# david-gimeno/tailored-avsr

Hardware: AMD Instinct MI355X
Metric: utterances/sec fwd+bwd, 12L tailored AV-Branchformer (Conv3d+ResNet-18 lip frontend, fusion, CTC+6L decoder), 4 s clips, batch 32/GPU (higher is better)
Workload: dtype f32

## Files before the change

profiles/gemm_trace.py:

```python
import ctypes as C
import os
import sys

ROOT = os.path.dirname(os.path.dirname(os.path.abspath(__file__)))
sys.path[:0] = [ROOT, os.path.join(ROOT, "tailored-avsr_amd")]
import numpy as np
import torch

from tavsr import _lib, ops

SHAPES = [("NT", 3168, 2048, 256, (4, 1)), ("NT", 3168, 2048, 256, (8, 1)), ("NT", 3168, 256, 2048, (4, 1)),
          ("NT", 3168, 256, 2048, (8, 4)), ("NT", 3168, 256, 2048, (8, 5)), ("NT", 3168, 256, 256, (4, 1)),
          ("NN", 3168, 256, 2048, (4, 1)), ("TN", 2048, 256, 3168, (4, 4))]


def pct(x):
    return " ".join(f"{np.percentile(x, q):7.2f}" for q in (0, 10, 50, 90, 100))


def main():
    L = _lib.lib()
    L.tavsr_gemm_trace_read.restype = C.c_int
    buf = np.zeros((1 << 15, 6), dtype=np.uint64)
    for mode, M, N, K, force in SHAPES:
        a = torch.randn(M, K, device="cuda")
        b = torch.randn(K, N, device="cuda")
        A = a.t().contiguous() if mode == "TN" else a
        B = b if mode != "NT" else b.t().contiguous()
        Cout = torch.empty(M, N, device="cuda")
        kw = dict(a_kmajor=mode == "TN", b_kmajor=mode != "NT")
        for _ in range(3):
            ops.gemm(M, N, K, A, A.stride(0), B, B.stride(0), Cout, N, force=force, **kw)
        torch.cuda.synchronize()
        L.tavsr_gemm_trace_read(buf.ctypes.data_as(C.c_void_p), buf.shape[0])
        ops.gemm(M, N, K, A, A.stride(0), B, B.stride(0), Cout, N, force=force, **kw)
        n = L.tavsr_gemm_trace_read(buf.ctypes.data_as(C.c_void_p), buf.shape[0])
        t = buf[:n, :4].astype(np.int64)
        t0 = t[:, 0].min()
        us = (t - t0) / 100.0
        hw = buf[:n, 4]
        xcc = (hw >> np.uint64(32)) & np.uint64(0xF)
        hwid = hw & np.uint64(0xFFFFFFFF)
        cu = (hwid >> np.uint64(8)) & np.uint64(0xF)
        sh = (hwid >> np.uint64(12)) & np.uint64(0x1)
        se = (hwid >> np.uint64(13)) & np.uint64(0x7)
        cuid = (xcc * np.uint64(8) + se) * np.uint64(32) + sh * np.uint64(16) + cu
        ncu = len(np.unique(cuid))
        per_cu = np.bincount(np.unique(cuid, return_inverse=True)[1])
        print(f"== {mode} M={M} N={N} K={K} cfg/split={force}: {n} workgroups on {ncu} CUs "
              f"(per CU min/med/max {per_cu.min()}/{int(np.median(per_cu))}/{per_cu.max()}), span {us[:, 3].max():.2f} us")
        print(f"   percentiles            {'p0':>7} {'p10':>7} {'p50':>7} {'p90':>7} {'p100':>7}")
        print(f"   start offset           {pct(us[:, 0])}")
        print(f"   prologue (first tile)  {pct(us[:, 1] - us[:, 0])}")
        print(f"   K loop                 {pct(us[:, 2] - us[:, 1])}")
        print(f"   epilogue               {pct(us[:, 3] - us[:, 2])}")
        print(f"   lifetime               {pct(us[:, 3] - us[:, 0])}")
        print(f"   end                    {pct(us[:, 3])}")
        cyc = buf[:n, 5].astype(np.float64)
        loop_us = np.maximum(us[:, 2] - us[:, 1], 1e-3)
        nk = max(1, (K // force[1]) // 32 - 1)
        print(f"   K-loop cycles/K-step   {pct(cyc / nk)}   shader clock GHz {pct(cyc / loop_us / 1e3)}", flush=True)


if __name__ == "__main__":
    main()
```

tailored-avsr_amd/csrc/gemm.hip:

```cpp
#include <algorithm>
#include <type_traits>

#include <cstdlib>
#include "common.h"

namespace tavsr {

typedef float f32x16 __attribute__((ext_vector_type(16)));

struct GemmArgs {
  tavsr_gemm_desc d;
  int kchunk;
  int nsplit;
  int tiles_m, tiles_n;
  int vec_epi;
  int zmap;
};

template <int V>
__global__ __launch_bounds__(256) void splitk_epilogue_kernel(const GemmArgs args) {
  const tavsr_gemm_desc& d = args.d;
  const int64_t mn = (int64_t)d.M * d.N;
  const int nbatch = d.nb1 * d.nb2;
  const int64_t i = ((int64_t)blockIdx.x * 256 + threadIdx.x) * V;
  const int z = blockIdx.y, z1 = z / d.nb2, z2 = z % d.nb2;
  if (d.a_rowsum && z == 0 && i < d.M) {
    const float* rs = d.ws + (int64_t)args.nsplit * nbatch * mn;
    for (int q = 0; q < V && i + q < d.M; ++q) {
      float v = 0.f;
      for (int s = 0; s < args.nsplit; ++s) v += rs[(int64_t)s * d.M + i + q];
      d.a_rowsum[i + q] = d.alpha * v;
    }
  }
  if (i >= mn) return;
  const int m = (int)(i / d.N), n = (int)(i % d.N);
  float v[V];
#pragma unroll
  for (int q = 0; q < V; ++q) v[q] = 0.f;
  const float* p = d.ws + (int64_t)z * mn + i;
#pragma unroll 4
  for (int s = 0; s < args.nsplit; ++s) {
    if (V == 4) {
      const float4 t = *reinterpret_cast<const float4*>(p + (int64_t)s * nbatch * mn);
      v[0] += t.x; v[1 % V] += t.y; v[2 % V] += t.z; v[3 % V] += t.w;
    } else {
      v[0] += p[(int64_t)s * nbatch * mn];
    }
  }
  const int64_t o = z1 * d.sC1 + z2 * d.sC2 + (int64_t)m * d.ldc + n;
  const int64_t ro = z1 * d.sR1 + z2 * d.sR2 + (int64_t)m * d.ldr + n;
  uint32_t keep[4] = {1u, 1u, 1u, 1u};
  float inv_keep = 1.f;
  if (V == 4 && d.drop_p > 0.f) {
    const uint64_t sd = d.drop_seed[0], ctr = (d.drop_offset >> 2) + (uint64_t)(i >> 2);
// ... 68 lines not shown
        if (gk < K) {
          const float* p = g + (int64_t)gk * ld + gr;
          if (VEC && gr + 3 < nrows) {
            val = *reinterpret_cast<const float4*>(p);
          } else {
            if (gr + 0 < nrows) val.x = p[0];
            if (gr + 1 < nrows) val.y = p[1];
            if (gr + 2 < nrows) val.z = p[2];
            if (gr + 3 < nrows) val.w = p[3];
          }
        }
      } else {
        if (gr < nrows) {
          const float* p = g + (int64_t)gr * ld + gk;
          if (VEC && gk + 3 < K) {
            val = *reinterpret_cast<const float4*>(p);
          } else {
            if (gk + 0 < K) val.x = p[0];
            if (gk + 1 < K) val.y = p[1];
            if (gk + 2 < K) val.z = p[2];
            if (gk + 3 < K) val.w = p[3];
          }
        }
      }
      r[i] = val;
    }
  }
  __device__ static __forceinline__ void store(float* __restrict__ s, int tid, const float4 (&r)[NV]) {
#pragma unroll
    for (int i = 0; i < NV; ++i) {
      int row, k;
      coords(tid + i * NT, row, k);
      *reinterpret_cast<float4*>(s + (KMAJOR ? k * T::LD + row : row * T::LD + k)) = r[i];
    }
  }
};

template <int ROWS, int BK, bool KMAJOR>
__device__ __forceinline__ void read_frag(const float* __restrict__ s, int row, int g, int lk, float (&f)[4]) {
  using T = Tile<ROWS, BK, KMAJOR>;
  if (KMAJOR) {
    const float* p = s + (g * 8 + 4 * lk) * T::LD + row;
#pragma unroll
    for (int j = 0; j < 4; ++j) f[j] = p[j * T::LD];
  } else {
    const float4 v = *reinterpret_cast<const float4*>(s + row * T::LD + g * 8 + 4 * lk);
    f[0] = v.x; f[1] = v.y; f[2] = v.z; f[3] = v.w;
  }
}

struct PosMajor {
  int n, H, W;
  int uni, base, rp;
  __device__ __forceinline__ void pos(int v, int& y, int& x) const {
    const int Hi = max(H - 2, 0), Wi = max(W - 2, 0), Hb = H - Hi, Wb = W - Wi;
    int u = v;
    if (u < Hi * Wi) { y = u / Wi + 1; x = u % Wi + 1; return; }
    u -= Hi * Wi;
    if (u < Hi * Wb) { y = u / Wb + 1; x = (u % Wb) ? W - 1 : 0; return; }
    u -= Hi * Wb;
    if (u < Hb * Wi) { y = (u / Wi) ? H - 1 : 0; x = u % Wi + 1; return; }
    u -= Hb * Wi;
    y = (u / Wb) ? H - 1 : 0;
    x = (u % Wb) ? W - 1 : 0;
  }
  __device__ __forceinline__ uint32_t taps(int y, int x) const {
    uint32_t mk = 0;
#pragma unroll
    for (int tap = 0; tap < 9; ++tap)
      mk |= (uint32_t)((unsigned)(y + tap / 3 - 1) < (unsigned)H && (unsigned)(x + tap % 3 - 1) < (unsigned)W) << tap;
    return mk;
  }
  __device__ __forceinline__ int row(int r) const {
    if (uni) return (r - base) * (H * W) + rp;
    const int v = r / n;
    int y, x;
    pos(v, y, x);
    return (r - v * n) * (H * W) + y * W + x;
  }
};

template <int TM, int TN, bool PM = false>
__device__ __forceinline__ void finish_tile(const tavsr_gemm_desc& d, int nsplit, f32x16 (&acc)[TM][TN],
                                            float (&asum)[TM], bool want_rowsum, int m0, int n0, int wm, int wn, int lr,
                                            int lk, int z1, int z2, int64_t coff, int zidx, const float* bias_pre = nullptr,
                                            const PosMajor* pm = nullptr) {
  if (want_rowsum) {
#pragma unroll
    for (int i = 0; i < TM; ++i) asum[i] += __shfl_xor(asum[i], 32, 64);
  }

  if (nsplit > 1) {
    const int64_t mn = (int64_t)d.M * d.N;
    const int nbatch = gridDim.y;
    float* slab = d.ws + ((int64_t)zidx * nbatch + blockIdx.y) * mn;
    float* rsum0 = d.ws + (int64_t)nsplit * nbatch * mn;
#pragma unroll
    for (int j = 0; j < TN; ++j) {
      const int n = n0 + wn * TN * 32 + j * 32 + lr;
      if (n >= d.N) continue;
#pragma unroll
      for (int i = 0; i < TM; ++i) {
        const int mb = m0 + wm * TM * 32 + i * 32 + 4 * lk;
#pragma unroll
        for (int r = 0; r < 16; ++r) {
          const int m = mb + (r & 3) + 8 * (r >> 2);
          if (m < d.M) slab[(int64_t)(PM ? pm->row(m) : m) * d.N + n] = acc[i][j][r];
        }
      }
    }
    if (want_rowsum && lk == 0) {
#pragma unroll
      for (int i = 0; i < TM; ++i) {
        const int m = m0 + wm * TM * 32 + i * 32 + lr;
        if (m < d.M) rsum0[(int64_t)zidx * d.M + m] = asum[i];
      }
    }
    return;
  }

  if (want_rowsum && lk == 0) {
#pragma unroll
    for (int i = 0; i < TM; ++i) {
      const int m = m0 + wm * TM * 32 + i * 32 + lr;
      if (m < d.M) d.a_rowsum[m] = d.alpha * asum[i];
    }
  }
  float* C = d.C + coff;
  float* Z = d.Z ? d.Z + coff : nullptr;
  const float* R = d.R ? d.R + z1 * d.sR1 + z2 * d.sR2 : nullptr;
  const float* DZ = d.DZ ? d.DZ + coff : nullptr;
#pragma unroll
  for (int j = 0; j < TN; ++j) {
// ... 808 lines not shown
      float* r0 = red + ((kw - 1) * WM * WN + w2) * PER * 64 + lane;
#pragma unroll
      for (int i = 0; i < TM; ++i)
#pragma unroll
        for (int j = 0; j < TN; ++j)
#pragma unroll
          for (int r = 0; r < 16; ++r) r0[((i * TN + j) * 16 + r) * 64] = acc[i][j][r];
#pragma unroll
      for (int i = 0; i < TM; ++i) rsum[(((kw - 1) * WM * WN + w2) * TM + i) * 64 + lane] = asum[i];
    }
    __syncthreads();
    if (kw > 0) return;
#pragma unroll
    for (int s2 = 0; s2 < KW - 1; ++s2) {
      const float* r0 = red + (s2 * WM * WN + w2) * PER * 64 + lane;
#pragma unroll
      for (int i = 0; i < TM; ++i)
#pragma unroll
        for (int j = 0; j < TN; ++j)
#pragma unroll
          for (int r = 0; r < 16; ++r) acc[i][j][r] += r0[((i * TN + j) * 16 + r) * 64];
#pragma unroll
      for (int i = 0; i < TM; ++i) asum[i] += rsum[((s2 * WM * WN + w2) * TM + i) * 64 + lane];
    }
  }
  if (KW == 1 && vec_epi) {
    static_assert(KW > 1 || BM * BN <= S * STAGE, "the output tile image must fit in the staging ring");
    if (want_rowsum) {
#pragma unroll
      for (int i = 0; i < TM; ++i) asum[i] += __shfl_xor(asum[i], 32, 64);
      if (lk == 0) {
#pragma unroll
        for (int i = 0; i < TM; ++i) {
          const int m = m0 + wm * TM * 32 + i * 32 + lr;
          if (m < d.M) {
            if (nsplit > 1) (d.ws + (int64_t)nsplit * gridDim.y * d.M * d.N)[(int64_t)zidx * d.M + m] = asum[i];
            else d.a_rowsum[m] = d.alpha * asum[i];
          }
        }
      }
    }
    finish_tile_vec<BM, BN, NT, TM, TN, PM && CONV == 1>(d, nsplit, acc, smem, m0, n0, wm, wn, lr, lk, z1, z2, coff, tid, zidx, &pm);
  } else {
    finish_tile<TM, TN, PM && CONV == 1>(d, nsplit, acc, asum, want_rowsum, m0, n0, wm, wn, lr, lk, z1, z2, coff, zidx, bpre, &pm);
  }
#ifdef TAVSR_GEMM_TRACE
  __builtin_amdgcn_s_waitcnt(0);
  TAVSR_TRACE_AT(3)
  if (tid == 0) {
    unsigned int slot = atomicAdd(&g_trace_n, 1u);
    if (slot < (unsigned)kTraceMax) {
      for (int i = 0; i < 4; ++i) g_trace[slot][i] = tr_t[i];
      g_trace[slot][4] = ((unsigned long long)__builtin_amdgcn_s_getreg((31 << 11) | 20) << 32) | __builtin_amdgcn_s_getreg((31 << 11) | 4);
      g_trace[slot][5] = tr_c[2] - tr_c[1];
    }
  }
#endif
}

__device__ __forceinline__ int xcd_remap(int bid, int nwg) {
  const int xcd = bid & 7, q = nwg >> 3, r = nwg & 7;
  return (xcd < r ? xcd * (q + 1) : r * (q + 1) + (xcd - r) * q) + (bid >> 3);
}

template <int BM, int BN, int WM, int WN, int S, int MINW, bool AK, bool BKM, int KW = 1, int CONV = 0, bool PM = false>
__global__ __launch_bounds__(WM* WN * KW * 64, MINW)
void gemm_glds_kernel(const GemmArgs args) {
  int bid = xcd_remap(blockIdx.x, gridDim.x), zidx = blockIdx.z;
  if (args.zmap) {
    const int tiles = gridDim.x, l = blockIdx.x + tiles * blockIdx.z, j = l >> 3;
    zidx = (l & 7) + 8 * (j / tiles);
    bid = j % tiles;
  }
  glds_tile<BM, BN, WM, WN, S, AK, BKM, KW, CONV, PM>(args.d, args.kchunk, args.nsplit, args.tiles_n, bid, args.vec_epi != 0, zidx);
}

constexpr int kMaxGroup = 12;
struct GroupArgs {
  tavsr_gemm_desc d[kMaxGroup];
  int tile_start[kMaxGroup + 1];
  int tiles_n[kMaxGroup];
  int n;
  int vec_epi;
};

template <int BM, int BN, int WM, int WN, int S, int MINW, bool AK, bool BKM>
__global__ __launch_bounds__(WM* WN * 64, MINW)
void gemm_glds_grouped_kernel(const GroupArgs g) {
  const int bid = xcd_remap(blockIdx.x, gridDim.x);
  int pi = 0;
#pragma unroll
  for (int i = 1; i < kMaxGroup; ++i)
    if (i < g.n && bid >= g.tile_start[i]) pi = i;
  glds_tile<BM, BN, WM, WN, S, AK, BKM>(g.d[pi], g.d[pi].K, 1, g.tiles_n[pi], bid - g.tile_start[pi], g.vec_epi != 0, 0);
}

struct Cfg {
  int bm, bn, wm, wn, stages;
};
static const Cfg kCfgs[] = {
    {128, 128, 2, 2, 3},
    {128, 128, 2, 4, 3},
    {128, 64, 2, 2, 3},
    {64, 128, 2, 2, 3},
    {64, 64, 2, 2, 3},
    {64, 64, 2, 2, 4},
    {128, 64, 2, 2, 4},
    {64, 64, 2, 2, 3},
    {64, 64, 2, 2, 2},
};
constexpr int kNumCfgs = sizeof(kCfgs) / sizeof(kCfgs[0]);
constexpr int kFallbackCfg = 9;

template <typename F>
static int launch_layout(const tavsr_gemm_desc& d, F&& f) {
  if (!d.a_kmajor && !d.b_kmajor) return f(std::false_type{}, std::false_type{});
  if (!d.a_kmajor && d.b_kmajor) return f(std::false_type{}, std::true_type{});
  if (d.a_kmajor && d.b_kmajor) return f(std::true_type{}, std::true_type{});
  return f(std::true_type{}, std::false_type{});
}

struct LnTail {
  const float* gamma; const float* beta; float eps; float* out; int64_t ld;
};
static const LnTail* g_ln_tail = nullptr;
// ... 51 lines not shown
      const float a = x[q].x - mean, b = x[q].y - mean, c = x[q].z - mean, e = x[q].w - mean;
      sq += (a * a + b * b) + (c * c + e * e);
    }
  }
  const float rstd = rsqrtf(wave_sum(sq) / (float)d.N + ln.eps);
#pragma unroll
  for (int q = 0; q < Q; ++q) {
    const int c4 = lane + 64 * q;
    if (c4 < n4) {
      const float4 g = *reinterpret_cast<const float4*>(ln.gamma + 4 * c4), b = *reinterpret_cast<const float4*>(ln.beta + 4 * c4);
      *reinterpret_cast<float4*>(ln.out + (int64_t)m * ln.ld + 4 * c4) =
          make_float4((x[q].x - mean) * rstd * g.x + b.x, (x[q].y - mean) * rstd * g.y + b.y, (x[q].z - mean) * rstd * g.z + b.z,
                      (x[q].w - mean) * rstd * g.w + b.w);
    }
  }
}

static int launch_epilogue(const GemmArgs& a, hipStream_t s) {
  const tavsr_gemm_desc& d = a.d;
  if (g_ln_tail) {
    hipLaunchKernelGGL(epilogue_ln_kernel, dim3(cdiv(d.M, 4)), dim3(256), 0, s, a, *g_ln_tail);
    TAVSR_LAUNCH_CHECK();
    return TAVSR_OK;
  }
  if (a.nsplit > 1) {
    const int64_t mn = (int64_t)d.M * d.N;
    if (d.N % 4 == 0)
      hipLaunchKernelGGL(splitk_epilogue_kernel<4>, dim3(cdiv(mn / 4, 256), d.nb1 * d.nb2), dim3(256), 0, s, a);
    else
      hipLaunchKernelGGL(splitk_epilogue_kernel<1>, dim3(cdiv(mn, 256), d.nb1 * d.nb2), dim3(256), 0, s, a);
    TAVSR_LAUNCH_CHECK();
  }
  return TAVSR_OK;
}

template <int BM, int BN, int WM, int WN, int S, int MINW, int KW = 1>
static int launch_glds(const tavsr_gemm_desc& d, int nsplit, int kchunk, hipStream_t s) {
  GemmArgs a{d, kchunk, nsplit, cdiv(d.M, BM), cdiv(d.N, BN), (int)vec_epi_ok(d)};
  dim3 grid(a.tiles_m * a.tiles_n, d.nb1 * d.nb2, nsplit);
  int rc = launch_layout(d, [&](auto ak, auto bk) {
    hipLaunchKernelGGL((gemm_glds_kernel<BM, BN, WM, WN, S, MINW, decltype(ak)::value, decltype(bk)::value, KW>), grid,
                       dim3(WM * WN * KW * 64), 0, s, a);
    TAVSR_LAUNCH_CHECK();
    return (int)TAVSR_OK;
  });
  return rc ? rc : launch_epilogue(a, s);
}

static bool conv_pm(const tavsr_gemm_desc& d) {
  return d.conv_posmajor && (d.conv_mode == 1 || d.conv_mode == 2) && d.conv_stride <= 1 && (d.conv_taps == 0 || d.conv_taps == 9) &&
         (d.conv_mode == 2 || !d.a_rowsum);
}

static int launch_conv(const tavsr_gemm_desc& d, int nsplit, int kchunk, hipStream_t s) {
  const int ve = (int)vec_epi_ok(d);
  constexpr int wide = 1;
  constexpr int dw_wide = 1;
  constexpr int zmap_on = 1;
  const int zmap = zmap_on && (d.conv_mode == 2 || d.conv_mode == 5 || d.conv_mode == 7) && nsplit >= 8 && nsplit % 8 == 0;
  if (d.conv_mode == 6 || d.conv_mode == 7) {
    GemmArgs a6{d, kchunk, nsplit, cdiv(d.M, 64), cdiv(d.N, 64), ve, zmap};
    const dim3 grid6(a6.tiles_m * a6.tiles_n, 1, nsplit);
    constexpr int st3 = 2;
    constexpr int tile128 = 0;
    if (d.conv_mode == 6 && tile128) {
      GemmArgs a7{d, kchunk, nsplit, cdiv(d.M, 128), cdiv(d.N, 64), ve, 0};
      hipLaunchKernelGGL((gemm_glds_kernel<128, 64, 2, 2, 2, 3, false, false, 1, 6>), dim3(a7.tiles_m * a7.tiles_n, 1, 1), dim3(256), 0, s, a7);
      TAVSR_LAUNCH_CHECK();
      return TAVSR_OK;
    }
    if (d.conv_mode == 6 && st3 == 3)
      hipLaunchKernelGGL((gemm_glds_kernel<64, 64, 2, 2, 3, 3, false, false, 1, 6>), grid6, dim3(256), 0, s, a6);
    else if (d.conv_mode == 6)
      hipLaunchKernelGGL((gemm_glds_kernel<64, 64, 2, 2, 2, 5, false, false, 1, 6>), grid6, dim3(256), 0, s, a6);
    else if (st3 == 3)
      hipLaunchKernelGGL((gemm_glds_kernel<64, 64, 2, 2, 3, 3, true, true, 1, 7>), grid6, dim3(256), 0, s, a6);
    else
      hipLaunchKernelGGL((gemm_glds_kernel<64, 64, 2, 2, 2, 5, true, true, 1, 7>), grid6, dim3(256), 0, s, a6);
    TAVSR_LAUNCH_CHECK();
    return launch_epilogue(a6, s);
  }
  if (d.conv_mode == 4 || d.conv_mode == 5) {
    GemmArgs a4{d, kchunk, nsplit, cdiv(d.M, 64), cdiv(d.N, 64), ve, zmap};
    const dim3 grid4(a4.tiles_m * a4.tiles_n, 1, nsplit);
    if (d.conv_mode == 4)
      hipLaunchKernelGGL((gemm_glds_kernel<64, 64, 2, 2, 2, 5, false, false, 1, 4>), grid4, dim3(256), 0, s, a4);
    else
      hipLaunchKernelGGL((gemm_glds_kernel<64, 64, 2, 2, 2, 5, true, true, 1, 5>), grid4, dim3(256), 0, s, a4);
    TAVSR_LAUNCH_CHECK();
    return launch_epilogue(a4, s);
  }
  const bool pm = conv_pm(d) && d.conv_mode == 1, pm2 = conv_pm(d) && d.conv_mode == 2;
  if (d.conv_mode == 1 && !d.b_kmajor && nsplit == 1 && wide && d.N % 128 == 0) {
    GemmArgs a2{d, kchunk, nsplit, cdiv(d.M, 64), cdiv(d.N, 128), (int)vec_epi_ok(d)};
    if (pm)
      hipLaunchKernelGGL((gemm_glds_kernel<64, 128, 2, 2, 2, 3, false, false, 1, 1, true>), dim3(a2.tiles_m * a2.tiles_n, 1, 1), dim3(256), 0, s, a2);
    else
      hipLaunchKernelGGL((gemm_glds_kernel<64, 128, 2, 2, 2, 3, false, false, 1, 1>), dim3(a2.tiles_m * a2.tiles_n, 1, 1), dim3(256), 0, s, a2);
    TAVSR_LAUNCH_CHECK();
    return TAVSR_OK;
  }
  if (d.conv_mode == 2 && dw_wide && d.M % 128 == 0) {
    GemmArgs a2{d, kchunk, nsplit, cdiv(d.M, 128), cdiv(d.N, 64), (int)vec_epi_ok(d), zmap};
    if (pm2)
      hipLaunchKernelGGL((gemm_glds_kernel<128, 64, 2, 2, 2, 3, true, true, 1, 2, true>), dim3(a2.tiles_m * a2.tiles_n, 1, nsplit), dim3(256), 0, s, a2);
    else
      hipLaunchKernelGGL((gemm_glds_kernel<128, 64, 2, 2, 2, 3, true, true, 1, 2>), dim3(a2.tiles_m * a2.tiles_n, 1, nsplit), dim3(256), 0, s, a2);
    TAVSR_LAUNCH_CHECK();
    return launch_epilogue(a2, s);
  }
  GemmArgs a{d, kchunk, nsplit, cdiv(d.M, 64), cdiv(d.N, 64), ve, zmap};
  dim3 grid(a.tiles_m * a.tiles_n, 1, nsplit);
  if (pm && !d.b_kmajor)
    hipLaunchKernelGGL((gemm_glds_kernel<64, 64, 2, 2, 2, 5, false, false, 1, 1, true>), grid, dim3(256), 0, s, a);
  else if (pm)
    hipLaunchKernelGGL((gemm_glds_kernel<64, 64, 2, 2, 2, 5, false, true, 1, 1, true>), grid, dim3(256), 0, s, a);
  else if (d.conv_mode == 1 && !d.b_kmajor)
    hipLaunchKernelGGL((gemm_glds_kernel<64, 64, 2, 2, 2, 5, false, false, 1, 1>), grid, dim3(256), 0, s, a);
  else if (d.conv_mode == 1)
    hipLaunchKernelGGL((gemm_glds_kernel<64, 64, 2, 2, 2, 5, false, true, 1, 1>), grid, dim3(256), 0, s, a);
  else if (pm2)
    hipLaunchKernelGGL((gemm_glds_kernel<64, 64, 2, 2, 2, 5, true, true, 1, 2, true>), grid, dim3(256), 0, s, a);
  else
    hipLaunchKernelGGL((gemm_glds_kernel<64, 64, 2, 2, 2, 5, true, true, 1, 2>), grid, dim3(256), 0, s, a);
  TAVSR_LAUNCH_CHECK();
  return launch_epilogue(a, s);
}

static int launch_fallback(const tavsr_gemm_desc& d, bool vec, int nsplit, int kchunk, hipStream_t s) {
  GemmArgs a{d, kchunk, nsplit, cdiv(d.M, 64), cdiv(d.N, 64), 0};
  dim3 grid(a.tiles_m * a.tiles_n, d.nb1 * d.nb2, nsplit);
  int rc = launch_layout(d, [&](auto ak, auto bk) {
    if (vec)
      hipLaunchKernelGGL((gemm_kernel<64, 64, 32, 2, 2, 2, 4, decltype(ak)::value, decltype(bk)::value, true>), grid,
                         dim3(256), 0, s, a);
    else
      hipLaunchKernelGGL((gemm_kernel<64, 64, 32, 2, 2, 2, 4, decltype(ak)::value, decltype(bk)::value, false>), grid,
                         dim3(256), 0, s, a);
    TAVSR_LAUNCH_CHECK();
    return (int)TAVSR_OK;
  });
  return rc ? rc : launch_epilogue(a, s);
}

static int launch_tail(const tavsr_gemm_desc& d, int nsplit, int kchunk, hipStream_t s) {
  GemmArgs a{d, kchunk, nsplit, cdiv(d.M, 64), cdiv(d.N, 64), (int)vec_epi_ok(d)};
  dim3 grid(a.tiles_m * a.tiles_n, d.nb1 * d.nb2, nsplit);
  int rc = launch_layout(d, [&](auto ak, auto bk) {
    hipLaunchKernelGGL((gemm_glds_kernel<64, 64, 2, 2, 2, 5, decltype(ak)::value, decltype(bk)::value, 1, 3>), grid, dim3(256), 0, s, a);
    TAVSR_LAUNCH_CHECK();
    return (int)TAVSR_OK;
  });
  return rc ? rc : launch_epilogue(a, s);
}

static int launch(int cfg, const tavsr_gemm_desc& d, bool vec, int nsplit, int kchunk, hipStream_t s) {
  switch (cfg) {
    case 0: return launch_glds<128, 128, 2, 2, 3, 1>(d, nsplit, kchunk, s);
    case 1: return launch_glds<128, 128, 2, 4, 3, 2>(d, nsplit, kchunk, s);
    case 2: return launch_glds<128, 64, 2, 2, 3, 2>(d, nsplit, kchunk, s);
    case 3: return launch_glds<64, 128, 2, 2, 3, 2>(d, nsplit, kchunk, s);
    case 4: return launch_glds<64, 64, 2, 2, 3, 3>(d, nsplit, kchunk, s);
    case 5: return launch_glds<64, 64, 2, 2, 4, 2>(d, nsplit, kchunk, s);
    case 6: return launch_glds<128, 64, 2, 2, 4, 1>(d, nsplit, kchunk, s);
    case 7: return launch_glds<64, 64, 2, 2, 3, 4, 2>(d, nsplit, kchunk, s);
    case 8: return launch_glds<64, 64, 2, 2, 2, 5>(d, nsplit, kchunk, s);
    default: return launch_fallback(d, vec, nsplit, kchunk, s);
  }
}

// ... 263 lines not shown
extern "C" int tavsr_gemm_grouped(const tavsr_gemm_desc* descs, int32_t n, tavsr_stream_t stream) {
  using namespace tavsr;
  TAVSR_REQUIRE(descs != nullptr && n >= 1 && n <= kMaxGroup, TAVSR_EINVAL, "tavsr_gemm_grouped: 1..%d problems", kMaxGroup);
  GroupArgs g;
  g.n = n;
  int total = 0;
  for (int i = 0; i < n; ++i) {
    tavsr_gemm_desc d = descs[i];
    if (d.nb1 <= 0) d.nb1 = 1;
    if (d.nb2 <= 0) d.nb2 = 1;
    TAVSR_REQUIRE(d.A && d.B && d.C && d.M > 0 && d.N > 0 && d.K > 0, TAVSR_EINVAL, "tavsr_gemm_grouped: bad problem %d", i);
    TAVSR_REQUIRE(d.a_kmajor == descs[0].a_kmajor && d.b_kmajor == descs[0].b_kmajor, TAVSR_EUNSUPPORTED,
                  "tavsr_gemm_grouped: all problems must share one layout");
    TAVSR_REQUIRE(d.nb1 * d.nb2 == 1 && d.drop_p == 0.f, TAVSR_EUNSUPPORTED, "tavsr_gemm_grouped: unbatched problems without epilogue dropout only");
    const bool vec = aligned16(d.A) && aligned16(d.B) && d.lda % 4 == 0 && d.ldb % 4 == 0;
    TAVSR_REQUIRE(glds_ok(d, vec), TAVSR_EUNSUPPORTED,
                  "tavsr_gemm_grouped: problem %d needs the predicated kernel (alignment / K %% 32 / rows %% 4)", i);
    if (d.R == nullptr) { d.ldr = 0; d.sR1 = d.sR2 = 0; }
    g.d[i] = d;
    g.tile_start[i] = total;
    g.tiles_n[i] = cdiv(d.N, 64);
    total += cdiv(d.M, 64) * g.tiles_n[i];
  }
  for (int i = n; i <= kMaxGroup; ++i) g.tile_start[i] = total;
  g.vec_epi = 1;
  for (int i = 0; i < n; ++i) g.vec_epi &= (int)vec_epi_ok(g.d[i]);
  hipStream_t s = static_cast<hipStream_t>(stream);
  int rc = launch_layout(descs[0], [&](auto ak, auto bk) {
    hipLaunchKernelGGL((gemm_glds_grouped_kernel<64, 64, 2, 2, 2, 5, decltype(ak)::value, decltype(bk)::value>), dim3(total),
                       dim3(256), 0, s, g);
    TAVSR_LAUNCH_CHECK();
    return (int)TAVSR_OK;
  });
  return rc;
}

extern "C" int tavsr_gemm_tune(const tavsr_gemm_desc* dp, int32_t cfg, int32_t nsplit, tavsr_stream_t stream) {
  return tavsr::run(dp, cfg, nsplit, static_cast<hipStream_t>(stream));
}

extern "C" int64_t tavsr_gemm_ws(const tavsr_gemm_desc* dp) {
  using namespace tavsr;
  if (!dp) return 0;
  tavsr_gemm_desc d = *dp;
  if (d.nb1 <= 0) d.nb1 = 1;
  if (d.nb2 <= 0) d.nb2 = 1;
  if (d.M <= 0 || d.N <= 0) return 0;
  const bool vec = aligned16(d.A) && aligned16(d.B) && d.lda % 4 == 0 && d.ldb % 4 == 0 && d.sA1 % 4 == 0 &&
                   d.sA2 % 4 == 0 && d.sB1 % 4 == 0 && d.sB2 % 4 == 0;
  Plan p = d.conv_mode != 0 ? plan_conv(d, true) : plan(d, true, glds_ok(d, vec) || tail_ok(d, vec));
  return ws_floats_for(d, p.nsplit);
}

#ifdef TAVSR_GEMM_TRACE
extern "C" int tavsr_gemm_trace_read(unsigned long long* out, int max_rows) {
  unsigned int n = 0;
  if (hipDeviceSynchronize() != hipSuccess) return -1;
  if (hipMemcpyFromSymbol(&n, HIP_SYMBOL(tavsr::g_trace_n), sizeof(n)) != hipSuccess) return -1;
  int rows = (int)(n < (unsigned)tavsr::kTraceMax ? n : tavsr::kTraceMax);
  if (rows > max_rows) rows = max_rows;
  if (rows > 0 && hipMemcpyFromSymbol(out, HIP_SYMBOL(tavsr::g_trace), (size_t)rows * 6 * sizeof(unsigned long long)) != hipSuccess) return -1;
  n = 0;
  if (hipMemcpyToSymbol(HIP_SYMBOL(tavsr::g_trace_n), &n, sizeof(n)) != hipSuccess) return -1;
  return rows;
}
#endif
```

tailored-avsr_amd/tavsr/ops.py:

```python
from __future__ import annotations

import ctypes as C
import os
from typing import Optional, Sequence

import torch

from . import _lib as L
from ._lib import ACT, AttnDesc, GemmDesc, check, lib, ptr, require_cuda, stream

f32 = torch.float32


def empty(*shape, like: Optional[torch.Tensor] = None, dtype=f32, device=None):
    dev = like.device if like is not None else (device if device is not None else "cuda")
    return torch.empty(shape, dtype=dtype, device=dev)


_addr = L.addr


class GemmProfile:

    def __init__(self, by_shape: bool = False):
# ... 1402 lines not shown
    dx = torch.empty_like(x)
    dg, db = empty(Cn, like=x), empty(Cn, like=x)
    ws = empty(lib().tavsr_bn_ws(M, Cn), like=x)
    check(lib().tavsr_bn_bwd_pooled(ptr(dpool), ptr(idx), ptr(x), ptr(mean), ptr(rstd), ptr(gamma), ptr(beta), ptr(dx), ptr(dg), ptr(db), N,
                                    H, W, Cn, ACT[act], ptr(ws), stream()), "tavsr_bn_bwd_pooled")
    return dx, dg, db


def maxpool3x3s2_fwd(x, N, H, W, Cn):
    Ho, Wo = conv_out(H, 3, 2, 1), conv_out(W, 3, 2, 1)
    y = empty(N * Ho * Wo, Cn, like=x)
    idx = torch.empty((N * Ho * Wo, Cn), dtype=torch.uint8, device=x.device)
    check(lib().tavsr_maxpool3x3s2_fwd(ptr(x), ptr(y), ptr(idx), N, H, W, Cn, stream()), "tavsr_maxpool3x3s2_fwd")
    return y, idx, Ho, Wo


def bn_act_maxpool3x3s2_fwd(z, mean, rstd, gamma, beta, act, N, H, W, Cn):
    Ho, Wo = conv_out(H, 3, 2, 1), conv_out(W, 3, 2, 1)
    require_cuda(z, mean, rstd, gamma, beta)
    y = empty(N * Ho * Wo, Cn, like=z)
    idx = torch.empty((N * Ho * Wo, Cn), dtype=torch.uint8, device=z.device)
    check(lib().tavsr_bn_act_maxpool3x3s2_fwd(ptr(z), ptr(mean), ptr(rstd), ptr(gamma), ptr(beta), ACT[act], ptr(y), ptr(idx), N, H, W, Cn,
                                              stream()), "tavsr_bn_act_maxpool3x3s2_fwd")
    return y, idx, Ho, Wo


def maxpool3x3s2_bwd(dy, idx, N, H, W, Cn):
    dx = empty(N * H * W, Cn, like=dy)
    check(lib().tavsr_maxpool3x3s2_bwd(ptr(dy), ptr(idx), ptr(dx), N, H, W, Cn, stream()), "tavsr_maxpool3x3s2_bwd")
    return dx


def avgpool_fwd(x, N, P, Cn):
    y = empty(N, Cn, like=x)
    check(lib().tavsr_avgpool_fwd(ptr(x), ptr(y), N, P, Cn, stream()), "tavsr_avgpool_fwd")
    return y


def avgpool_bwd(dy, N, P, Cn):
    dx = empty(N * P, Cn, like=dy)
    check(lib().tavsr_avgpool_bwd(ptr(dy), ptr(dx), N, P, Cn, stream()), "tavsr_avgpool_bwd")
    return dx


def conv_wflip(w2d, cout, cin):
    require_cuda(w2d)
    out = empty(cin, 9 * cout, like=w2d)
    check(lib().tavsr_conv_wflip(ptr(w2d), ptr(out), cout, cin, stream()), "tavsr_conv_wflip")
    return out


CONV_TAPSKIP = os.environ.get("TAVSR_CONV_TAPSKIP", "1") != "0"
CONV_TAPSKIP_MAXPOS = int(os.environ.get("TAVSR_CONV_TAPSKIP_MAXPOS", "36"))


def _tapskip(H, W, stride=1, taps=9, pad0=False):
    return int(CONV_TAPSKIP and stride == 1 and taps == 9 and not pad0 and H * W <= CONV_TAPSKIP_MAXPOS)


def conv3x3_fwd(x, w2d, H, W, stride=1, taps=9, pad0=False, bias=None, act=None):
    M, cin = x.shape
    cout = w2d.shape[0]
    if pad0:
        assert taps == 9
        Ho, Wo = (H - 3) // stride + 1, (W - 3) // stride + 1
    else:
        Ho, Wo = (H - 1) // stride + 1, (W - 1) // stride + 1
    Mo = M // (H * W) * Ho * Wo
    z = empty(Mo, cout, like=x)
    gemm(Mo, cout, taps * cin, x, cin, w2d, taps * cin, z, cout, conv=(1, H, W, cin, stride, 90 if pad0 else taps, _tapskip(H, W, stride, taps, pad0)),
         bias=bias, act=act)
    return z


def conv3x3_dx(dz, wflip, H, W, res=None):
    M, cout = dz.shape
    cin = wflip.shape[0]
    dx = empty(M, cin, like=dz)
    gemm(M, cin, 9 * cout, dz, cout, wflip, 9 * cout, dx, cin, conv=(1, H, W, cout, 0, 0, _tapskip(H, W)), R=res, ldr=0 if res is None else cin)
    return dx


def conv3x3_dw(dz, x, H, W, stride=1, taps=9, pad0=False, bias_grad=False):
    M, cout = dz.shape
    cin = x.shape[1]
    dw = empty(cout, taps * cin, like=dz)
    gb = empty(cout, like=dz) if bias_grad else None
    gemm(cout, taps * cin, M, dz, cout, x, cin, dw, taps * cin, a_kmajor=True, b_kmajor=True,
         conv=(2, H, W, cin, stride, 90 if pad0 else taps, _tapskip(H, W, stride, taps, pad0)), a_rowsum=gb)
    return (dw, gb) if bias_grad else dw


def fill_(t, value):
    require_cuda(t)
    assert t.is_contiguous()
    check(lib().tavsr_fill(ptr(t), value, t.numel(), stream()), "tavsr_fill")
    return t


def copy2d(src, dst):
    require_cuda(src, dst)
    assert src.shape == dst.shape and src.dim() == 2 and src.stride(1) == 1 and dst.stride(1) == 1
    check(lib().tavsr_copy2d(ptr(src), src.stride(0), ptr(dst), dst.stride(0), src.shape[0], src.shape[1], stream()), "tavsr_copy2d")
    return dst


def stft_frames(wav, window, T, n_fft, hop, center=True):
    B, N = wav.shape
    require_cuda(wav, window)
    frames = empty(B * T, n_fft, like=wav)
# ... 411 lines not shown
```

Baseline: 389.9.

## Schedule tap-skip conv GEMM tiles heaviest-first and reorder weight-gradient tiles by tap

Builds a host-side tile order for position-major tap-skip conv GEMMs that sorts M-tile runs by their active tap count, so the tiles with the most K work are dispatched first. A small struct with this order is passed to the kernel, which remaps the block index through it. For the split-K weight-gradient path it also permutes tiles by tap rank. Both aim to reduce tail imbalance from uneven per-tile K work, at the cost of extra kernel argument size, index arithmetic per block, and a cached host computation. Also adds profiling scripts and packs K-step counts into the trace data.

Measured after the change: 411.1, median of 6. 1.05x the previous value.

```diff
diff --git a/profiles/conv_launches.py b/profiles/conv_launches.py
--- /dev/null
+++ b/profiles/conv_launches.py
@@ -0,0 +1,69 @@
+import csv
+import os
+import sys
+from collections import defaultdict
+
+ROOT = os.path.dirname(os.path.dirname(os.path.abspath(__file__)))
+sys.path[:0] = [ROOT, os.path.join(ROOT, "tailored-avsr_amd")]
+N_IMG = 3200
+LAYERS = (("layer 4", 3, 3, 512), ("layer 3", 6, 6, 256))
+FLAGS = (0, 3, 1)
+
+
+def labels():
+    out = []
+    for name, H, W, Cc in LAYERS:
+        out += [f"{name} forward NT {N_IMG * H * W}x{Cc}x{9 * Cc} posmajor={f}" for f in FLAGS]
+        out += [f"{name} wgrad TN {Cc}x{9 * Cc}x{N_IMG * H * W} posmajor={f}" for f in FLAGS]
+    return out
+
+
+def run():
+    import torch
+    from tavsr import ops
+    for name, H, W, Cc in LAYERS:
+        M, K = N_IMG * H * W, 9 * Cc
+        x = torch.randn(M, Cc, device="cuda")
+        w = torch.randn(Cc, K, device="cuda") / K ** 0.5
+        dz = torch.randn(M, Cc, device="cuda")
+        z = torch.empty(M, Cc, device="cuda")
+        dw = torch.empty(Cc, K, device="cuda")
+        for f in FLAGS:
+            for _ in range(2):
+                ops.gemm(M, Cc, K, x, Cc, w, K, z, Cc, conv=(1, H, W, Cc, 1, 9, f))
+        for f in FLAGS:
+            for _ in range(2):
+                ops.gemm(Cc, K, M, dz, Cc, x, Cc, dw, K, a_kmajor=True, b_kmajor=True, conv=(2, H, W, Cc, 1, 9, f))
+        torch.cuda.synchronize()
+
+
+def summarise(path):
+    rows = defaultdict(dict)
+    names = {}
+    with open(path) as f:
+        for r in csv.DictReader(f):
+            if "gemm_glds_kernel" not in r["Kernel_Name"]:
+                continue
+            d = int(r["Dispatch_Id"])
+            rows[d][r["Counter_Name"]] = rows[d].get(r["Counter_Name"], 0.0) + float(r["Counter_Value"])
+            names[d] = r["Kernel_Name"]
+    ids = sorted(rows)
+    lab = labels()
+    assert len(ids) == 2 * len(lab), (len(ids), len(lab))
+    counters = sorted({c for v in rows.values() for c in v})
+    print(f"{'launch':58s} " + " ".join(f"{c:>24s}" for c in counters) + ("   L2 hit rate" if "TCC_HIT_sum" in counters else ""))
+    for i, name in enumerate(lab):
+        v = rows[ids[2 * i + 1]]
+        extra = f"   {v['TCC_HIT_sum'] / max(1.0, v['TCC_HIT_sum'] + v['TCC_MISS_sum']):.3f}" if "TCC_HIT_sum" in v else ""
+        if "SQ_VALU_MFMA_BUSY_CYCLES" in v and "SQ_BUSY_CU_CYCLES" in v:
+            extra += f"   MFMA busy / CU busy {v['SQ_VALU_MFMA_BUSY_CYCLES'] / max(1.0, v['SQ_BUSY_CU_CYCLES']):.3f}"
+        if "SQ_WAIT_ANY" in v and "SQ_WAVE_CYCLES" in v:
+            extra += f"   wait / wave cycles {v['SQ_WAIT_ANY'] / max(1.0, v['SQ_WAVE_CYCLES']):.3f}"
+        print(f"{name:58s} " + " ".join(f"{v.get(c, float('nan')):24.0f}" for c in counters) + extra)
+
+
+if __name__ == "__main__":
+    if len(sys.argv) > 2 and sys.argv[1] == "--summarise":
+        summarise(sys.argv[2])
+    else:
+        run()
diff --git a/profiles/gemm_trace.py b/profiles/gemm_trace.py
--- a/profiles/gemm_trace.py
+++ b/profiles/gemm_trace.py
@@ -18,7 +18,66 @@
     return " ".join(f"{np.percentile(x, q):7.2f}" for q in (0, 10, 50, 90, 100))
 
 
+def read_trace(L, buf):
+    n = L.tavsr_gemm_trace_read(buf.ctypes.data_as(C.c_void_p), buf.shape[0])
+    t = buf[:n, :4].astype(np.int64)
+    us = (t - t[:, 0].min()) / 100.0
+    xcc = ((buf[:n, 4] >> np.uint64(32)) & np.uint64(0xF)).astype(np.int64)
+    cyc = (buf[:n, 5] & np.uint64((1 << 40) - 1)).astype(np.float64)
+    nk = (buf[:n, 5] >> np.uint64(40)).astype(np.int64)
+    return n, us, xcc, cyc, nk
+
+
+def conv_main():
+    L = _lib.lib()
+    L.tavsr_gemm_trace_read.restype = C.c_int
+    buf = np.zeros((1 << 15, 6), dtype=np.uint64)
+    n_img = 3200
+    for name, H, W, Cc in (("layer 4", 3, 3, 512), ("layer 3", 6, 6, 256)):
+        M, K = n_img * H * W, 9 * Cc
+        x = torch.randn(M, Cc, device="cuda")
+        w = torch.randn(Cc, K, device="cuda") / K ** 0.5
+        dz = torch.randn(M, Cc, device="cuda")
+        z = torch.empty(M, Cc, device="cuda")
+        dw = torch.empty(Cc, K, device="cuda")
+        launches = [(f"{name} forward NT {M}x{Cc}x{K} conv_posmajor={f}", f,
+                     lambda f=f: ops.gemm(M, Cc, K, x, Cc, w, K, z, Cc, conv=(1, H, W, Cc, 1, 9, f))) for f in (0, 3, 1)]
+        launches += [(f"{name} weight gradient TN {Cc}x{K}x{M} conv_posmajor={f}", f,
+                      lambda f=f: ops.gemm(Cc, K, M, dz, Cc, x, Cc, dw, K, a_kmajor=True, b_kmajor=True, conv=(2, H, W, Cc, 1, 9, f)))
+                     for f in (0, 3, 1)]
+        for title, f, run in launches:
+            for _ in range(3):
+                run()
+            torch.cuda.synchronize()
+            L.tavsr_gemm_trace_read(buf.ctypes.data_as(C.c_void_p), buf.shape[0])
+            e0, e1 = torch.cuda.Event(enable_timing=True), torch.cuda.Event(enable_timing=True)
+            e0.record()
+            run()
+            e1.record()
+            torch.cuda.synchronize()
+            n, us, xcc, cyc, nk = read_trace(L, buf)
+            life = np.maximum(us[:, 3] - us[:, 0], 1e-3)
+            outside = 1.0 - (us[:, 2] - us[:, 1]) / life
+            print(f"== {title}: {n} workgroups, span {us[:, 3].max():.1f} us (events {e0.elapsed_time(e1) * 1e3:.1f} us, traced kernels "
+                  f"only), outside the K loop: {100 * outside.mean():.1f} % of a tile's life (prologue {np.mean(us[:, 1] - us[:, 0]):.2f} us, "
+                  f"epilogue {np.mean(us[:, 3] - us[:, 2]):.2f} us of {life.mean():.1f} us)")
+            print("   per XCD: tiles, K-steps, first start, last end (us)")
+            for xc in np.unique(xcc):
+                s = xcc == xc
+                print(f"     xcd {xc}: {s.sum():5d} {nk[s].sum():8d} {us[s, 0].min():8.1f} {us[s, 3].max():8.1f}")
+            print("   per tile class (K-steps executed): tiles, cycles per K-step p10 / p50 / p90, K loop us p50, by quartile of start time p50")
+            cps = cyc / np.maximum(nk - 1, 1)
+            for k in np.unique(nk)[::-1]:
+                s = nk == k
+                order = np.argsort(us[s, 0])
+                q = [np.median(cps[s][part]) for part in np.array_split(order, 4) if len(part)]
+                print(f"     {k:4d}: {s.sum():5d}  {np.percentile(cps[s], 10):7.0f} {np.median(cps[s]):7.0f} {np.percentile(cps[s], 90):7.0f}  "
+                      f"{np.median(us[s, 2] - us[s, 1]):7.1f}   " + " ".join(f"{v:7.0f}" for v in q), flush=True)
+
+
 def main():
+    if "--conv" in sys.argv[1:]:
+        return conv_main()
     L = _lib.lib()
     L.tavsr_gemm_trace_read.restype = C.c_int
     buf = np.zeros((1 << 15, 6), dtype=np.uint64)
@@ -56,7 +115,7 @@
         print(f"   epilogue               {pct(us[:, 3] - us[:, 2])}")
         print(f"   lifetime               {pct(us[:, 3] - us[:, 0])}")
         print(f"   end                    {pct(us[:, 3])}")
-        cyc = buf[:n, 5].astype(np.float64)
+        cyc = (buf[:n, 5] & np.uint64((1 << 40) - 1)).astype(np.float64)
         loop_us = np.maximum(us[:, 2] - us[:, 1], 1e-3)
         nk = max(1, (K // force[1]) // 32 - 1)
         print(f"   K-loop cycles/K-step   {pct(cyc / nk)}   shader clock GHz {pct(cyc / loop_us / 1e3)}", flush=True)
diff --git a/tailored-avsr_amd/csrc/gemm.hip b/tailored-avsr_amd/csrc/gemm.hip
--- a/tailored-avsr_amd/csrc/gemm.hip
+++ b/tailored-avsr_amd/csrc/gemm.hip
@@ -1,5 +1,6 @@
 #include <algorithm>
 #include <type_traits>
+#include <vector>
 
 #include <cstdlib>
 #include "common.h"
@@ -174,8 +175,8 @@
 struct PosMajor {
   int n, H, W;
   int uni, base, rp;
-  __device__ __forceinline__ void pos(int v, int& y, int& x) const {
-    const int Hi = max(H - 2, 0), Wi = max(W - 2, 0), Hb = H - Hi, Wb = W - Wi;
+  __host__ __device__ __forceinline__ void pos(int v, int& y, int& x) const {
+    const int Hi = H > 2 ? H - 2 : 0, Wi = W > 2 ? W - 2 : 0, Hb = H - Hi, Wb = W - Wi;
     int u = v;
     if (u < Hi * Wi) { y = u / Wi + 1; x = u % Wi + 1; return; }
     u -= Hi * Wi;
@@ -186,7 +187,7 @@
     y = (u / Wb) ? H - 1 : 0;
     x = (u % Wb) ? W - 1 : 0;
   }
-  __device__ __forceinline__ uint32_t taps(int y, int x) const {
+  __host__ __device__ __forceinline__ uint32_t taps(int y, int x) const {
     uint32_t mk = 0;
 #pragma unroll
     for (int tap = 0; tap < 9; ++tap)
@@ -201,6 +202,41 @@
     return (r - v * n) * (H * W) + y * W + x;
   }
 };
+
+constexpr int kOrdRuns = 80;
+struct TileOrder {
+  int nruns;
+  int start[kOrdRuns];
+  int cum[kOrdRuns + 1];
+  int w[kOrdRuns];
+};
+
+__host__ __device__ inline void tile_order_map(const TileOrder& o, int b, int tiles_m, int tiles_n, int& mt, int& nt) {
+  const int per = 8 * tiles_n;
+  const int g = b / per, j = b - g * per, s0 = 8 * g;
+  int r0 = 0;
+  while (r0 + 1 < o.nruns && o.cum[r0 + 1] <= s0) ++r0;
+  bool uniform = s0 + 8 <= tiles_m;
+  if (uniform) {
+    int r7 = r0;
+    while (r7 + 1 < o.nruns && o.cum[r7 + 1] <= s0 + 7) ++r7;
+    uniform = o.w[r7] == o.w[r0];
+  }
+  const int s = s0 + (uniform ? (j & 7) : j / tiles_n);
+  nt = uniform ? (j >> 3) : j % tiles_n;
+  int r = r0;
+  while (r + 1 < o.nruns && o.cum[r + 1] <= s) ++r;
+  mt = o.start[r] + s - o.cum[r];
+}
+
+__host__ __device__ inline int dw_tile_order(int q, int tiles_m, int tiles_n, int H, int W) {
+  if (tiles_n % 9 != 0) return q;
+  const int tpt = tiles_n / 9, per = tiles_m * tpt;
+  const int rank = q / per, rem = q - rank * per;
+  const unsigned long long taps = (H - 1) * W >= H * (W - 1) ? 0x862053714ull : 0x862071534ull;
+  const int tap = (int)((taps >> (4 * rank)) & 15);
+  return (rem / tpt) * tiles_n + tap * tpt + rem % tpt;
+}
 
 template <int TM, int TN, bool PM = false>
 __device__ __forceinline__ void finish_tile(const tavsr_gemm_desc& d, int nsplit, f32x16 (&acc)[TM][TN],
@@ -1115,7 +1151,7 @@
     if (slot < (unsigned)kTraceMax) {
       for (int i = 0; i < 4; ++i) g_trace[slot][i] = tr_t[i];
       g_trace[slot][4] = ((unsigned long long)__builtin_amdgcn_s_getreg((31 << 11) | 20) << 32) | __builtin_amdgcn_s_getreg((31 << 11) | 4);
-      g_trace[slot][5] = tr_c[2] - tr_c[1];
+      g_trace[slot][5] = ((tr_c[2] - tr_c[1]) & 0xFFFFFFFFFFull) | ((unsigned long long)nk << 40);
     }
   }
 #endif
@@ -1126,14 +1162,32 @@
   return (xcd < r ? xcd * (q + 1) : r * (q + 1) + (xcd - r) * q) + (bid >> 3);
 }
 
+struct GemmArgsOrd {
+  GemmArgs g;
+  TileOrder ord;
+};
+__device__ __forceinline__ const GemmArgs& common_args(const GemmArgs& a) { return a; }
+__device__ __forceinline__ const GemmArgs& common_args(const GemmArgsOrd& a) { return a.g; }
+
 template <int BM, int BN, int WM, int WN, int S, int MINW, bool AK, bool BKM, int KW = 1, int CONV = 0, bool PM = false>
 __global__ __launch_bounds__(WM* WN * KW * 64, MINW)
-void gemm_glds_kernel(const GemmArgs args) {
+void gemm_glds_kernel(const std::conditional_t<PM && CONV == 1, GemmArgsOrd, GemmArgs> xargs) {
+  const GemmArgs& args = common_args(xargs);
   int bid = xcd_remap(blockIdx.x, gridDim.x), zidx = blockIdx.z;
+  if constexpr (PM && CONV == 1) {
+    if (xargs.ord.nruns > 0) {
+      int mt, nt;
+      tile_order_map(xargs.ord, blockIdx.x, args.tiles_m, args.tiles_n, mt, nt);
+      bid = mt * args.tiles_n + nt;
+    }
+  }
   if (args.zmap) {
     const int tiles = gridDim.x, l = blockIdx.x + tiles * blockIdx.z, j = l >> 3;
     zidx = (l & 7) + 8 * (j / tiles);
     bid = j % tiles;
+    if constexpr (PM && CONV == 2) {
+      if (!(args.d.conv_posmajor & 2)) bid = dw_tile_order(bid, args.tiles_m, args.tiles_n, args.d.conv_H, args.d.conv_W);
+    }
   }
   glds_tile<BM, BN, WM, WN, S, AK, BKM, KW, CONV, PM>(args.d, args.kchunk, args.nsplit, args.tiles_n, bid, args.vec_epi != 0, zidx);
 }
@@ -1291,6 +1345,47 @@
          (d.conv_mode == 2 || !d.a_rowsum);
 }
 
+static void tile_order_build(const tavsr_gemm_desc& d, int BM, int nsplit, TileOrder& o) {
+  o.nruns = 0;
+  const int P = d.conv_H * d.conv_W;
+  if (nsplit != 1 || (d.conv_posmajor & 2) || P <= 0 || d.M < P) return;
+  struct Key { int H, W, M, BM; };
+  static thread_local Key last{0, 0, 0, 0};
+  static thread_local TileOrder last_o;
+  if (last.H == d.conv_H && last.W == d.conv_W && last.M == d.M && last.BM == BM) { o = last_o; return; }
+  PosMajor pm{};
+  pm.H = d.conv_H; pm.W = d.conv_W; pm.n = d.M / P;
+  std::vector<uint32_t> tp(P);
+  for (int v = 0; v < P; ++v) {
+    int y, x;
+    pm.pos(v, y, x);
+    tp[v] = pm.taps(y, x);
+  }
+  struct Run { int start, len, w; };
+  std::vector<Run> runs;
+  const int tiles_m = cdiv(d.M, BM);
+  for (int i = 0; i < tiles_m; ++i) {
+    const int vlo = (int)((int64_t)i * BM / pm.n);
+    const int vhi = std::min((int)(std::min<int64_t>((int64_t)i * BM + BM - 1, d.M - 1) / pm.n), P - 1);
+    uint32_t mk = 0;
+    for (int v = vlo; v <= vhi; ++v) mk |= tp[v];
+    const int w = __builtin_popcount(mk);
+    if (!runs.empty() && runs.back().w == w) ++runs.back().len;
+    else runs.push_back(Run{i, 1, w});
+    if ((int)runs.size() > kOrdRuns) return;
+  }
+  std::stable_sort(runs.begin(), runs.end(), [](const Run& a, const Run& b) { return a.w > b.w; });
+  int cum = 0;
+  for (size_t r = 0; r < runs.size(); ++r) {
+    o.start[r] = runs[r].start; o.cum[r] = cum; o.w[r] = runs[r].w;
+    cum += runs[r].len;
+  }
+  o.cum[runs.size()] = cum;
+  o.nruns = (int)runs.size();
+  last = Key{d.conv_H, d.conv_W, d.M, BM};
+  last_o = o;
+}
+
 static int launch_conv(const tavsr_gemm_desc& d, int nsplit, int kchunk, hipStream_t s) {
   const int ve = (int)vec_epi_ok(d);
   constexpr int wide = 1;
@@ -1332,9 +1427,11 @@
   const bool pm = conv_pm(d) && d.conv_mode == 1, pm2 = conv_pm(d) && d.conv_mode == 2;
   if (d.conv_mode == 1 && !d.b_kmajor && nsplit == 1 && wide && d.N % 128 == 0) {
     GemmArgs a2{d, kchunk, nsplit, cdiv(d.M, 64), cdiv(d.N, 128), (int)vec_epi_ok(d)};
-    if (pm)
-      hipLaunchKernelGGL((gemm_glds_kernel<64, 128, 2, 2, 2, 3, false, false, 1, 1, true>), dim3(a2.tiles_m * a2.tiles_n, 1, 1), dim3(256), 0, s, a2);
-    else
+    if (pm) {
+      GemmArgsOrd ao{a2, {}};
+      tile_order_build(d, 64, nsplit, ao.ord);
+      hipLaunchKernelGGL((gemm_glds_kernel<64, 128, 2, 2, 2, 3, false, false, 1, 1, true>), dim3(a2.tiles_m * a2.tiles_n, 1, 1), dim3(256), 0, s, ao);
+    } else
       hipLaunchKernelGGL((gemm_glds_kernel<64, 128, 2, 2, 2, 3, false, false, 1, 1>), dim3(a2.tiles_m * a2.tiles_n, 1, 1), dim3(256), 0, s, a2);
     TAVSR_LAUNCH_CHECK();
     return TAVSR_OK;
@@ -1350,11 +1447,14 @@
   }
   GemmArgs a{d, kchunk, nsplit, cdiv(d.M, 64), cdiv(d.N, 64), ve, zmap};
   dim3 grid(a.tiles_m * a.tiles_n, 1, nsplit);
-  if (pm && !d.b_kmajor)
-    hipLaunchKernelGGL((gemm_glds_kernel<64, 64, 2, 2, 2, 5, false, false, 1, 1, true>), grid, dim3(256), 0, s, a);
-  else if (pm)
-    hipLaunchKernelGGL((gemm_glds_kernel<64, 64, 2, 2, 2, 5, false, true, 1, 1, true>), grid, dim3(256), 0, s, a);
-  else if (d.conv_mode == 1 && !d.b_kmajor)
+  if (pm) {
+    GemmArgsOrd ao{a, {}};
+    tile_order_build(d, 64, nsplit, ao.ord);
+    if (!d.b_kmajor)
+      hipLaunchKernelGGL((gemm_glds_kernel<64, 64, 2, 2, 2, 5, false, false, 1, 1, true>), grid, dim3(256), 0, s, ao);
+    else
+      hipLaunchKernelGGL((gemm_glds_kernel<64, 64, 2, 2, 2, 5, false, true, 1, 1, true>), grid, dim3(256), 0, s, ao);
+  } else if (d.conv_mode == 1 && !d.b_kmajor)
     hipLaunchKernelGGL((gemm_glds_kernel<64, 64, 2, 2, 2, 5, false, false, 1, 1>), grid, dim3(256), 0, s, a);
   else if (d.conv_mode == 1)
     hipLaunchKernelGGL((gemm_glds_kernel<64, 64, 2, 2, 2, 5, false, true, 1, 1>), grid, dim3(256), 0, s, a);
@@ -1724,6 +1824,25 @@
   return ws_floats_for(d, p.nsplit);
 }
 
+extern "C" int tavsr_conv_tile_order(int H, int W, int images, int bm, int tiles_n, int32_t* tile_m, int32_t* tile_n, int max_blocks) {
+  using namespace tavsr;
+  if (H <= 0 || W <= 0 || images <= 0 || bm <= 0 || tiles_n <= 0) return 0;
+  tavsr_gemm_desc d{};
+  d.conv_H = H; d.conv_W = W; d.M = images * H * W; d.conv_posmajor = 1;
+  TileOrder o;
+  tile_order_build(d, bm, 1, o);
+  if (o.nruns == 0) return 0;
+  const int tiles_m = cdiv(d.M, bm), nwg = tiles_m * tiles_n;
+  for (int b = 0; b < nwg && b < max_blocks; ++b) tile_order_map(o, b, tiles_m, tiles_n, tile_m[b], tile_n[b]);
+  return nwg;
+}
+
+extern "C" int tavsr_conv_dw_tile_order(int H, int W, int tiles_m, int tiles_n, int32_t* tile, int max_tiles) {
+  if (H <= 0 || W <= 0 || tiles_m <= 0 || tiles_n <= 0) return 0;
+  for (int q = 0; q < tiles_m * tiles_n && q < max_tiles; ++q) tile[q] = tavsr::dw_tile_order(q, tiles_m, tiles_n, H, W);
+  return tiles_m * tiles_n;
+}
+
 #ifdef TAVSR_GEMM_TRACE
 extern "C" int tavsr_gemm_trace_read(unsigned long long* out, int max_rows) {
   unsigned int n = 0;
diff --git a/tailored-avsr_amd/tavsr/ops.py b/tailored-avsr_amd/tavsr/ops.py
--- a/tailored-avsr_amd/tavsr/ops.py
+++ b/tailored-avsr_amd/tavsr/ops.py
@@ -1478,10 +1478,12 @@
 
 CONV_TAPSKIP = os.environ.get("TAVSR_CONV_TAPSKIP", "1") != "0"
 CONV_TAPSKIP_MAXPOS = int(os.environ.get("TAVSR_CONV_TAPSKIP_MAXPOS", "36"))
+CONV_TILEORDER = os.environ.get("TAVSR_CONV_TILEORDER", "1") != "0"
 
 
 def _tapskip(H, W, stride=1, taps=9, pad0=False):
-    return int(CONV_TAPSKIP and stride == 1 and taps == 9 and not pad0 and H * W <= CONV_TAPSKIP_MAXPOS)
+    on = CONV_TAPSKIP and stride == 1 and taps == 9 and not pad0 and H * W <= CONV_TAPSKIP_MAXPOS
+    return (1 if CONV_TILEORDER else 3) if on else 0
 
 
 def conv3x3_fwd(x, w2d, H, W, stride=1, taps=9, pad0=False, bias=None, act=None):
```
